# batra-mlp-lab/visdial

Hardware: AMD Instinct MI355X
Metric: QA-rounds/sec training mn-att-ques-im-hist+disc (batch 20x10x100) (higher is better)
Workload: dtype f32 operands and results; the option recurrence multiplies the EXACT 3-way bf16 split of both operands (9 bf16 MFMA products per fp32 product, f32 accumulate: fp32-grade, errors at the f32 MFMA's own level) -- its two step kernels and its weight-gradient contraction; f32 MFMA (v_mfma_f32_32x32x2_f32

## Files before the change

visdial_amd/csrc/comm.hip:

```cpp
#include <dlfcn.h>

#include "common.h"
#include "rt_core.h"
#include "../../include/visdial_hip.h"

namespace {

struct NcclUniqueId { char internal[128]; };
typedef void* NcclComm;
typedef int NcclResult;
enum { kNcclFloat32 = 7, kNcclSum = 0 };

struct Rccl {
  void* lib = nullptr;
  NcclResult (*GetUniqueId)(NcclUniqueId*) = nullptr;
  NcclResult (*CommInitRank)(NcclComm*, int, NcclUniqueId, int) = nullptr;
  NcclResult (*CommDestroy)(NcclComm) = nullptr;
  NcclResult (*AllReduce)(const void*, void*, size_t, int, int, NcclComm, hipStream_t) = nullptr;
  NcclResult (*GroupStart)() = nullptr;
  NcclResult (*GroupEnd)() = nullptr;
  const char* (*GetErrorString)(NcclResult) = nullptr;
  NcclResult (*GetVersion)(int*) = nullptr;
};

// ... 150 lines not shown
int vd_comm_destroy(void) {
  if (!g.comm) return VD_OK;
  if (g.stream) (void)hipStreamSynchronize(g.stream);
  NcclResult r = g.api.CommDestroy(g.comm);
  release_local();
  if (r != 0) {
    vd_set_error("vd_comm_destroy: ncclCommDestroy -> %s", g.api.GetErrorString(r));
    return VD_ERR_HIP;
  }
  return VD_OK;
}

int vd_model_allreduce_grads(vd_model* m) {
  VdRange r("vd_model_allreduce_grads");
  VD_CHECK_ARG(m, "vd_model_allreduce_grads: null model");
  VD_CHECK_ARG(g.comm, "vd_model_allreduce_grads: no communicator (vd_comm_init first)");
  VD_CHECK_ARG(m->cur >= 0, "vd_model_allreduce_grads: no backward pass has been enqueued");
  int dev = -1;
  VD_HIP(hipGetDevice(&dev));
  VD_CHECK_ARG(dev == g.device, "vd_model_allreduce_grads: communicator lives on device %d, current device is %d", g.device, dev);
  int64_t lo = 0, hi = 0;
  int rc = vd_model_encoder_range(m, &lo, &hi);
  if (rc != VD_OK) return rc;
  const bool split = hi > lo && m->enc_grads_recorded;
  if (split) {
    VD_HIP(hipStreamWaitEvent(g.stream, m->ev_enc_grads, 0));
    VD_NCCL(g.api.AllReduce(m->G + lo, m->G + lo, (size_t)(hi - lo), kNcclFloat32, kNcclSum, g.comm, g.stream));
    VD_HIP(hipEventRecord(g.ev_b1, g.stream));
    VD_HIP(hipEventRecord(g.ev_tail_t, m->s_main));
  }
  g.timed = split;
  VD_HIP(hipEventRecord(g.ev_tail, m->s_main));
  VD_HIP(hipStreamWaitEvent(g.stream, g.ev_tail, 0));
  if (split) {
    VD_NCCL(g.api.GroupStart());
    NcclResult r = 0;
    if (lo > 0) r = g.api.AllReduce(m->G, m->G, (size_t)lo, kNcclFloat32, kNcclSum, g.comm, g.stream);
    if (r == 0 && m->numel > hi)
      r = g.api.AllReduce(m->G + hi, m->G + hi, (size_t)(m->numel - hi), kNcclFloat32, kNcclSum, g.comm, g.stream);
    NcclResult rend = g.api.GroupEnd();
    if (r != 0 || rend != 0) {
      vd_set_error("vd_model_allreduce_grads: bucket 2 -> %s", g.api.GetErrorString(r != 0 ? r : rend));
      return VD_ERR_HIP;
    }
  } else {
    VD_NCCL(g.api.AllReduce(m->G, m->G, (size_t)m->numel, kNcclFloat32, kNcclSum, g.comm, g.stream));
// ... 12 lines not shown
```

visdial_amd/csrc/rt_core.h:

```cpp
#pragma once
#include <math.h>
#include <stdarg.h>
#include <stdlib.h>
#include <string.h>

#include <algorithm>
#include <map>
#include <memory>
#include <numeric>
#include <random>
#include <string>
#include <vector>

#include "../../include/visdial_hip.h"
#include "common.h"
#include "paths.h"
#include "rt_switches.h"
#include "wgrad_plan.h"

static_assert(VD_OK == 0 && VD_ERR_ARG == -1, "rt_switches.h returns the two as literals: it includes no common.h");

int vd_lstm2_forward_p(const vd_lstm2_fwd_t* st, int nstacks, int H, int flags, hipStream_t stream);
int vd_lstm2_backward_p(const vd_lstm2_bwd_t* st, int nstacks, int H, int flags, hipStream_t stream);

int vd_img_drop_gather(const float* pre, const uint8_t* mask1, float* xdrop, int N, int R, int S2, int H, float scale, hipStream_t stream);
int vd_img_common_forward_p(const float* pre, const uint8_t* mask1, const float* xdrop, const float* Wc, const float* bc, const float* qc,
                            const uint8_t* mask2, float* iqc, int N, int R, int S2, int H, int Kc, float scale, int flags, hipStream_t stream);
int vd_img_tr_backward_p(const float* dz, const float* Wc, const float* p, const float* datt, const uint8_t* mask1, float* dpre, int N, int R,
                         int S2, int H, int Kc, float scale, int flags, hipStream_t stream);
int vd_img_common_wgrad_p(const float* dz, const float* pre, const uint8_t* mask1, const float* xdrop, float* dWc, int N, int R, int S2, int H,
                          int Kc, float scale, int flags, hipStream_t stream);

int vd_img_att_forward_p(const float* iqc, const float* wa, const float* ba, const float* pre, const uint8_t* mask1, const float* u0, float* p,
                         float* u1, int N, int R, int S2, int H, int Kc, float scale, const int32_t* cnt, hipStream_t stream);
int vd_img_att_backward_p(float* iqc_dz, const float* wa, const float* pre, const uint8_t* mask1, const uint8_t* mask2, const float* p,
                          const float* datt, float* dwa, float* dba, float* dqc, float* work, int N, int R, int S2, int H, int Kc, float scale,
                          const int32_t* cnt, hipStream_t stream);

int vd_mn_attention_round_p(const float* Q, int64_t q_ld, const float* Hm, float* P, float* hAtt, float* Qout, int B, int R, int r, int H,
                            hipStream_t stream);
int vd_hrea_attention_round_p(const float* sq, const float* sh, const float* Hm, float* P, float* att, int B, int R, int r, int H,
// ... 185 lines not shown
}

struct vd_model {
  vd_model_params p;
  int flags = 0;
  std::string enc_name, dec_name;
  std::vector<vdrt::Tensor> spec;
  std::map<std::string, int> index;
  long numel = 0;
  float *W = nullptr, *G = nullptr, *M = nullptr, *V = nullptr;
  std::map<std::string, vdrt::DevBuf> ws;
  std::map<std::string, vdrt::DevBuf> ext_masks;
  hipStream_t s_main = nullptr, s_side = nullptr;
  hipStream_t s_wg = nullptr;
  bool wg_active = false, wg_used = false;
  std::vector<vdrt::WgradProduct> wgrad;
  bool wgrad_open = false, wgrad_hold = false;
  std::vector<hipEvent_t> ev_pool;
  size_t ev_next = 0;
  hipEvent_t ev_enc_grads = nullptr;
  hipEvent_t ev_updated = nullptr;
  bool updated_recorded = false;
  bool enc_grads_recorded = false;
  hipEvent_t ev_loss = nullptr, ev_prof[6] = {nullptr, nullptr, nullptr, nullptr, nullptr, nullptr};
  bool training = true, streams = true, prof_valid = false;
  long step = 0;
  int adam_t = 0;
  double lr = 1e-3;
  vdrt::BatchSlot slot[2];
  int cur = -1, uploaded = -1;
  float* loss_host = nullptr;
  long loss_cap = 0, loss_n = 0;
  bool loss_is_sum = false;
  double loss_div = 0.0;
  std::unique_ptr<vdrt::Encoder> enc;
  std::unique_ptr<vdrt::Decoder> dec;
  float* scores = nullptr;
  float* gen_enc_out = nullptr;
  int gen_seq_len = 0;
  int N = 0, O = 0;
  long lhood_exec = -1, lhood_total = 0;
  bool step_live = false;
  bool use_im = false, use_hist = false, is_att = false, is_graph = false;
  vdrt::OptionCache ocache;
  vdrt::Switches sw;
  int rollout_max_words = 0;
// ... 30 lines not shown
}

template <class T>
int ws_get(vd_model* m, const std::string& key, size_t count, T** out) {
  void* p = nullptr;
  VD_TRY(dev_get(m->ws, key, count * sizeof(T), &p));
  *out = static_cast<T*>(p);
  return VD_OK;
}

inline void add_lstm(vd_model* m, const std::string& name, long D, long H) {
  m->spec.push_back(Tensor{name + ".W", 0, D + H, 4 * H, 1});
  m->spec.push_back(Tensor{name + ".b", 0, 1, 4 * H, 2});
}
inline void add_linear(vd_model* m, const std::string& name, long in, long out) {
  m->spec.push_back(Tensor{name + ".W", 0, out, in, 3});
  m->spec.push_back(Tensor{name + ".b", 0, 1, out, 4});
}
inline std::string hop_sfx(int i) { return i == 0 ? std::string() : std::to_string(i + 1); }

inline float* Wp(vd_model* m, const std::string& n) { return m->W + m->spec[m->index.at(n)].off; }
inline float* Gp(vd_model* m, const std::string& n) { return m->G + m->spec[m->index.at(n)].off; }

inline int fork_stream(vd_model* m, hipStream_t from, hipStream_t side) {
  if (side == from) return VD_OK;
  hipEvent_t e = m->ev_pool[m->ev_next++ % m->ev_pool.size()];
  VD_HIP(hipEventRecord(e, from));
  VD_HIP(hipStreamWaitEvent(side, e, 0));
  return VD_OK;
}
inline int join_stream(vd_model* m, hipStream_t side, hipStream_t to) { return fork_stream(m, side, to); }
inline hipStream_t side_stream(vd_model* m, hipStream_t cur) { return m->streams ? m->s_side : cur; }
inline int wg_fork(vd_model* m, hipStream_t cur, hipStream_t* out) {
  *out = cur;
  if (!m->wg_active || !m->s_wg) return VD_OK;
  VD_TRY(fork_stream(m, cur, m->s_wg));
  m->wg_used = true;
  *out = m->s_wg;
  return VD_OK;
}

constexpr int VD_WGRAD_CHUNKS = 768, VD_WGRAD_MIN_KSTEPS = 32;
inline void wgrad_begin(vd_model* m) {
  m->wgrad.clear();
  m->wgrad_open = true;
}
// ... 359 lines not shown
```

visdial_amd/csrc/rt_decoders.h:

```cpp
#pragma once
#include "rt_encoders.h"

namespace vdrt {

int option_cache_resolve(vd_model* m, BatchSlot& sl, const int32_t* options, long NO, int To, hipStream_t s);

struct Decoder {
  virtual ~Decoder() {}
  virtual void declare(vd_model* m) = 0;
  virtual int forward_backward(vd_model* m, BatchSlot& b, bool only_forward) = 0;
  virtual int retrieve(vd_model* m, BatchSlot& b) = 0;
  virtual int retrieve_lhood(vd_model*, BatchSlot&) {
    vd_set_error("vd_model_retrieve_lhood: the live-row log-likelihood head scores candidates of decoder 'gen'; this model's decoder is 'disc'");
    return VD_ERR_ARG;
  }
  virtual int gen_begin(vd_model*, const int32_t*, int) { return no_gen(); }
  virtual int gen_step(vd_model*, const int32_t*, float*) { return no_gen(); }
  virtual int gen_select(vd_model*, const int32_t*, int) { return no_gen(); }
  virtual int gen_beam_search(vd_model*, int, int, int, int, int32_t*, double*) { return no_gen(); }
  virtual int gen_sample(vd_model*, int, int, int, double, const double*, int32_t*, double*) { return no_gen(); }
  static int no_gen() {
    vd_set_error("sampling / beam search only for the generative decoder (model.lua:436-438)");
    return VD_ERR_STATE;
  }
// ... 20 lines not shown
               "state of the first: under training-mode dropout the passes would not describe one model; call vd_model_set_training(0) first",
               call);
  return VD_ERR_STATE;
}
inline int rollout_encode(vd_model* m, hipStream_t s, BatchSlot& b, int r, float** enc_out) {
  return m->sw.rollout_round ? m->enc->forward_round(m, s, b, r, enc_out) : m->enc->forward(m, s, b, enc_out);
}
struct HistRows {
  int32_t *tok, *tok_sorted, *inv;
  explicit HistRows(BatchSlot& b) : tok(b.h.tok), tok_sorted(b.h.sorted ? b.h.tok_sorted : nullptr), inv(b.h.sorted ? b.h.inv : nullptr) {}
};

#ifdef VD_PROBE_PHASES
inline hipEvent_t* probe_events() {
  static hipEvent_t e[6];
  static bool made = false;
  if (!made) { for (auto& x : e) (void)hipEventCreate(&x); made = true; }
  return e;
}
#define VD_PROBE_REC(i, stream) (void)hipEventRecord(probe_events()[i], stream)
#else
#define VD_PROBE_REC(i, stream)
#endif
struct Disc : Decoder {
  void declare(vd_model* m) override { add_lstm(m, "opt", m->p.embedSize, m->p.rnnHiddenSize); }
  struct OptStates {
    bool c16;
    float *table, *gates, *h, *c, *h_last;
    vd_bf16_bits *gates16, *h16;
    const float* optH;
  };
  int option_states(vd_model* m, const SeqTok& opt, OptStates* o) {
    const int NO = opt.N, To = opt.T;
    const long H = m->p.rnnHiddenSize, E = m->p.embedSize, V = m->p.vocabSize;
    hipStream_t s = m->s_main;
    VD_TRY(ws_get(m, "opt.table", (size_t)(V + 1) * 4 * H, &o->table));
    VD_TRY(ws_get(m, "opt.gates", (size_t)To * NO * 4 * H, &o->gates));
    VD_TRY(ws_get(m, "opt.h", (size_t)To * NO * H, &o->h));
    VD_TRY(ws_get(m, "opt.c", (size_t)To * NO * H, &o->c));
    float* Wopt = Wp(m, "opt.W");
    const int flags = m->flags;
    VD_TRY(vd_gemm_nn(Wp(m, "embed"), E, Wopt, 4 * H, Wp(m, "opt.b"), o->table, 4 * H, (int)V + 1, (int)(4 * H), (int)E, 0, s));
    o->c16 = (flags & VD_FLAG_BF16) && vd_lstm_c16_fits(NO, (int)H);
    o->gates16 = reinterpret_cast<vd_bf16_bits*>(o->gates);
    o->h16 = reinterpret_cast<vd_bf16_bits*>(o->h);
    o->h_last = nullptr;
    vd_bf16_bits* table16 = nullptr;
    if (o->c16) {
      float* t16;
      VD_TRY(ws_get(m, "opt.table16", (size_t)(V + 1) * 2 * H, &t16));
      VD_TRY(ws_get(m, "opt.h_last", (size_t)NO * H, &o->h_last));
      table16 = reinterpret_cast<vd_bf16_bits*>(t16);
      VD_TRY(vd_f32_to_bf16(o->table, table16, (V + 1) * 4 * H, s));
    }
    VD_HIP(hipEventRecord(m->ev_prof[0], s));
    {
      VdRange r("disc: option LSTM forward");
      if (o->c16) VD_TRY(vd_lstm_forward_c16(table16, 4 * H, opt.tok, Wopt + E * 4 * H, o->gates16, o->h16, o->h_last, o->c, To, NO, (int)H, s));
      else VD_TRY(vd_lstm_forward(o->table, 0, 4 * H, opt.tok, nullptr, Wopt + E * 4 * H, nullptr, nullptr, o->gates, o->h, o->c, To, NO, (int)H, flags, s));
    }
    VD_HIP(hipEventRecord(m->ev_prof[1], s));
    o->optH = o->c16 ? o->h_last : o->h + (long)(To - 1) * NO * H;
    return VD_OK;
  }
  int option_states_full(vd_model* m, BatchSlot& b, const OptStates& o, const float** optH) {
    *optH = o.optH;
    if (!b.opt_uid) return VD_OK;
    const long NOfull = (long)b.q.N * m->p.numOptions, H = m->p.rnnHiddenSize;
    float* full;
    VD_TRY(ws_get(m, "opt.h_full", (size_t)NOfull * H, &full));
    VD_TRY(vd_embed_gather(o.optH, b.opt_uid, nullptr, full, NOfull, (int)H, 1.f, m->s_main));
    *optH = full;
    return VD_OK;
  }
  int forward_backward(vd_model* m, BatchSlot& b, bool only_forward) override {
    VD_CHECK_ARG(b.opt.present, "decoder 'disc' needs batch.options");
    VD_CHECK_ARG(only_forward || b.has_gt, "training decoder 'disc' needs batch.answer_ind");
// ... 95 lines not shown
    VdRange rwg("disc: table gradient + dWh");
    VD_TRY(fork_stream(m, s, sd));
    if (!m->wgrad.empty()) {
      VD_TRY(wgrad_flush(m, b, sd));
      VD_HIP(hipEventRecord(m->ev_enc_grads, sd));
    }
    if (c16) VD_TRY(vd_segment_rowsum_acc_bf16(gates16, 4 * H, opt.tok, perm, (long)To * NO, (int)(4 * H), dtab, 4 * H, sd));
    else VD_TRY(vd_segment_rowsum_acc(gates, 4 * H, opt.tok, perm, (long)To * NO, (int)(4 * H), dtab, 4 * H, sd));
    VD_TRY(vd_colsum_acc(dtab, 4 * H, (int)V + 1, (int)(4 * H), Gp(m, "opt.b"), sd));
    VD_TRY(vd_gemm_tn_acc(Wp(m, "embed"), E, dtab, 4 * H, Gp(m, "opt.W"), 4 * H, (int)E, (int)(4 * H), (int)V + 1, 0, sd));
    VD_HIP(hipEventRecord(m->ev_prof[4], s));
    if (To > 1 && c16)
      VD_TRY(vd_gemm_tn_acc_bf16(h16, gates16 + (long)NO * 4 * H, Gp(m, "opt.W") + E * 4 * H, 4 * H, (int)H, (int)(4 * H), (To - 1) * NO, s));
    else if (To > 1)
      VD_TRY(vd_gemm_tn_acc(h, H, gates + (long)NO * 4 * H, 4 * H, Gp(m, "opt.W") + E * 4 * H, 4 * H, (int)H, (int)(4 * H), (To - 1) * NO,
                            flags & (VD_FLAG_BF16 | VD_FLAG_SPLIT9), s));
    VD_HIP(hipEventRecord(m->ev_prof[5], s));
    VD_TRY(vd_gemm_nt(dtab, 4 * H, Wopt, 4 * H, nullptr, Gp(m, "embed"), E, (int)V + 1, (int)E, (int)(4 * H), VD_ACT_NONE, 2, sd));
    VD_PROBE_REC(3, sd);
    VD_TRY(join_stream(m, sd, s));
    if (m->wg_used) VD_TRY(join_stream(m, m->s_wg, s));
    m->wg_active = m->wg_used = false;
    VD_PROBE_REC(4, s);
    return VD_OK;
  }
  int retrieve(vd_model* m, BatchSlot& b) override {
    if (m->sw.retrieve_rollout && m->use_hist) return retrieve_rollout(m, b);
    return forward_backward(m, b, true);
  }

  int retrieve_rollout(vd_model* m, BatchSlot& b) {
    VD_TRY(refuse_round_rollout_in_training(m, "vd_model_retrieve"));
    if (m->training) {
      vd_set_error("vd_model_retrieve: this model was created with VD_RETRIEVE_ROLLOUT = 1, and a rollout re-runs the encoder once per round: "
                   "under training-mode dropout the passes would not describe one model; call vd_model_set_training(0) first");
      return VD_ERR_STATE;
    }
    VD_CHECK_ARG(b.opt.present && !b.cached, "decoder 'disc' needs batch.options");
    const int N = b.q.N, O = m->p.numOptions, NOfull = N * O, NO = b.opt.N, R = m->p.maxQuesCount, B = N / R;
    const bool dedup = b.opt_uid != nullptr;
    VD_CHECK_ARG(dedup ? NO <= NOfull : NO == NOfull, "decoder 'disc': %d option rows for %d x %d candidates", NO, N, O);
    VD_CHECK_ARG(b.h.present && b.q.present && b.h.N == N && N == B * R && b.h.T >= b.q.T,
                 "vd_model_retrieve: VD_RETRIEVE_ROLLOUT = 1 needs the batch's history, Th >= Tq");
    const long H = m->p.rnnHiddenSize;
    hipStream_t s = m->s_main;
    hipStream_t sd = side_stream(m, s);
// ... 17 lines not shown
      if (r > 0) {
        VdRange rr("encoder forward");
        VD_TRY(rollout_encode(m, s, b, r, &enc_out));
      }
      VD_TRY(vd_score_ce(optH, enc_out, b.gt, scores, loss_rows, nullptr, nullptr, N, O, (int)H, 1.0f / N, s));
      if (r + 1 < R)
        VD_TRY(vd_disc_rollout_pick_p(scores, O, b.opt.tok, NO, b.opt.T, b.opt_uid, b.q.tok, b.q.T, B, R, r, hr.tok, hr.tok_sorted, hr.inv,
                                      b.h.T, s, m->sw.rollout_concat_end));
    }
    VD_TRY(stage_loss(m, loss_rows, N, false, s));
    m->scores = scores;
    m->prof_valid = false;
    return VD_OK;
  }

  int forward_cached(vd_model* m, BatchSlot& b, bool only_forward) {
    if (!only_forward || m->training) {
      vd_set_error("decoder 'disc': this batch was uploaded for cached evaluation (VD_OPTION_CACHE with training off) and carries only the "
                   "candidate rows the cache did not hold; upload it again after vd_model_set_training(1) for a training step");
      return VD_ERR_STATE;
    }
    OptionCache& oc = m->ocache;
    const int N = b.q.N, O = m->p.numOptions, NOfull = N * O, To = b.opt.T;
    const long H = m->p.rnnHiddenSize, E = m->p.embedSize, V = m->p.vocabSize;
    hipStream_t s = m->s_main;
    hipStream_t sd = side_stream(m, s);
    if (b.cache_stamp != oc.stamp) {
      VD_HIP(hipEventSynchronize(b.ready));
      VD_TRY(option_cache_resolve(m, b, b.opt_host.data(), NOfull, To, s));
      VD_HIP(hipStreamSynchronize(s));
    }
    const int U = b.opt.N;
    const long count = oc.index.size();
    VD_CHECK_ARG(b.opt_total == NOfull && (long)b.miss_keys.size() == (long)U * To && count <= oc.capacity,
                 "decoder 'disc': inconsistent cached batch (%d candidates, %d misses)", b.opt_total, U);
    if (oc.table_rows < count + U) {
      const long want = std::min(std::max(2 * oc.table_rows, VD_OPTION_CACHE_FIRST_ROWS), oc.capacity);
      const long rows = std::max(want, count + U);
      float* nt = nullptr;
      VD_HIP(hipMalloc((void**)&nt, (size_t)rows * H * sizeof(float)));
      if (oc.table) {
        if (count > 0) VD_HIP(hipMemcpyAsync(nt, oc.table, (size_t)count * H * sizeof(float), hipMemcpyDeviceToDevice, s));
        VD_HIP(hipStreamSynchronize(s));
        VD_HIP(hipFree(oc.table));
      }
      oc.table = nt;
      oc.table_rows = rows;
    }
    float *scores, *loss_rows, *full;
    VD_TRY(ws_get(m, "opt.scores", (size_t)N * O, &scores));
    VD_TRY(ws_get(m, "crit.loss_rows", (size_t)N, &loss_rows));
    VD_TRY(ws_get(m, "opt.h_full", (size_t)NOfull * H, &full));
    VD_TRY(fork_stream(m, s, sd));
    if (U > 0) {
      VdRange r("disc: option LSTM forward (state only, cache misses)");
      float *table, *h, *c;
      VD_TRY(ws_get(m, "opt.table", (size_t)(V + 1) * 4 * H, &table));
      VD_TRY(ws_get(m, "opt.h2", (size_t)2 * U * H, &h));
      VD_TRY(ws_get(m, "opt.c2", (size_t)2 * U * H, &c));
      float* Wopt = Wp(m, "opt.W");
      VD_TRY(vd_gemm_nn(Wp(m, "embed"), E, Wopt, 4 * H, Wp(m, "opt.b"), table, 4 * H, (int)V + 1, (int)(4 * H), (int)E, 0, s));
      VD_TRY(vd_lstm_forward(table, 0, 4 * H, b.opt.tok, nullptr, Wopt + E * 4 * H, nullptr, nullptr, nullptr, h, c, To, U, (int)H,
                             m->flags | VD_FLAG_STATE_ONLY, s));
      VD_HIP(hipMemcpyAsync(oc.table + count * H, h + (long)((To - 1) & 1) * U * H, (size_t)U * H * sizeof(float), hipMemcpyDeviceToDevice, s));
      const long fit = std::min<long>(U, oc.capacity - count);
      for (long i = 0; i < fit; ++i) oc.index.add(b.miss_keys.data() + (size_t)i * To);
    }
    ++oc.stamp;
    float* enc_out = nullptr;
    {
      VdRange r("encoder forward");
      VD_TRY(m->enc->forward(m, sd, b, &enc_out));
    }
    VD_TRY(join_stream(m, sd, s));
    VD_TRY(vd_embed_gather(oc.table, b.opt_uid, nullptr, full, NOfull, (int)H, 1.f, s));
    VD_TRY(vd_score_ce(full, enc_out, b.gt, scores, loss_rows, nullptr, nullptr, N, O, (int)H, 1.0f / N, s));
    VD_TRY(stage_loss(m, loss_rows, N, false, s));
    m->scores = scores;
    m->prof_valid = false;
    return VD_OK;
  }
};

struct Gen;
// ... 585 lines not shown
```

visdial_amd/csrc/runtime.hip:

```cpp
#include "rt_decoders.h"

using namespace vdrt;

vd_model::~vd_model() {}

namespace {

int upload_tokens(BatchSlot& sl, SeqTok& ss, const std::string& tag, const int32_t* rows_major, int N, int T, bool sorted, hipStream_t s,
                  int rollout_R = 0) {
  ss.T = T;
  ss.N = N;
  ss.present = true;
  ss.sorted = sorted;
  sl.wgrad_sig.clear();
  const size_t TN = (size_t)T * N;
  const size_t seg_at = (7 * TN + 2 * (size_t)N + T + 3) / 4 * 4, seg_ints = 4 * ((size_t)T + 1);
  const size_t total = sorted ? seg_at + 2 * seg_ints : TN;
  int32_t* stage = nullptr;
  VD_TRY(pin_get(sl.pinned, tag + ".stage", total * sizeof(int32_t), (void**)&stage));
  int32_t* tok = stage;
  std::vector<int> len(sorted ? N : 0);
  for (int n = 0; n < N; ++n) {
    int first = T;
    for (int t = 0; t < T; ++t) {
// ... 258 lines not shown
  m->ocache.capacity = sw.option_cache_rows;
  if (m->p.numAttentionLayers < 1 || has(en, "lf-att")) m->p.numAttentionLayers = 1;
  if (m->p.numLayers < 1) m->p.numLayers = 2;
  m->enc_name = encoder;
  m->dec_name = decoder;
  m->use_im = use_im;
  m->use_hist = has(en, "hist");
  m->is_att = is_att;
  m->is_graph = en.rfind("mn", 0) == 0 || en.rfind("lf-att", 0) == 0;
  m->lr = p->learningRate;
  m->streams = p->useStreams != 0;
  m->enc = std::move(enc);
  m->dec = std::move(dec);
  m->spec.push_back(Tensor{"embed", 0, p->vocabSize + 1, p->embedSize, 0});
  m->enc->declare(m);
  m->dec->declare(m);
  long off = 0;
  for (size_t i = 0; i < m->spec.size(); ++i) {
    m->spec[i].off = off;
    m->index[m->spec[i].name] = (int)i;
    off += (m->spec[i].numel() + 3) / 4 * 4;
  }
  m->numel = off;
  auto fail = [&](int rc) {
    vd_model_destroy(m);
    return rc;
  };
  for (float** v : {&m->W, &m->G, &m->M, &m->V}) {
    if (hipMalloc((void**)v, off * sizeof(float)) != hipSuccess) {
      vd_set_error("vd_model_create: hipMalloc of %ld floats failed", off);
      return fail(VD_ERR_HIP);
    }
    (void)hipMemset(*v, 0, off * sizeof(float));
  }
  int least = 0, greatest = 0;
  (void)hipDeviceGetStreamPriorityRange(&least, &greatest);
  if (hipStreamCreateWithPriority(&m->s_main, hipStreamNonBlocking, least) != hipSuccess) return fail(VD_ERR_HIP);
  if (hipStreamCreateWithPriority(&m->s_side, hipStreamNonBlocking, greatest) != hipSuccess) return fail(VD_ERR_HIP);
  if (least - greatest >= 2 &&
      hipStreamCreateWithPriority(&m->s_wg, hipStreamNonBlocking, (least + greatest) / 2) != hipSuccess)
    return fail(VD_ERR_HIP);
  m->ev_pool.resize(64);
  for (auto& e : m->ev_pool)
    if (hipEventCreateWithFlags(&e, hipEventDisableTiming) != hipSuccess) return fail(VD_ERR_HIP);
  if (hipEventCreateWithFlags(&m->ev_loss, hipEventDisableTiming) != hipSuccess) return fail(VD_ERR_HIP);
  if (hipEventCreateWithFlags(&m->ev_enc_grads, hipEventDisableTiming) != hipSuccess) return fail(VD_ERR_HIP);
// ... 40 lines not shown
    }
  delete m;
}

int64_t vd_model_num_tensors(const vd_model* m) { return m ? (int64_t)m->spec.size() : 0; }
int64_t vd_model_flat_size(const vd_model* m) { return m ? m->numel : 0; }

int vd_model_tensor_info(const vd_model* m, int64_t i, char* name64, int64_t* offset, int64_t* rows, int64_t* cols) {
  VD_CHECK_ARG(m && i >= 0 && i < (int64_t)m->spec.size(), "vd_model_tensor_info: bad index");
  const Tensor& t = m->spec[i];
  if (name64) {
    strncpy(name64, t.name.c_str(), 63);
    name64[63] = 0;
  }
  if (offset) *offset = t.off;
  if (rows) *rows = t.rows;
  if (cols) *cols = t.cols;
  return VD_OK;
}

int vd_model_flat_pointers(vd_model* m, float** W, float** dW, float** adam_m, float** adam_v) {
  VD_CHECK_ARG(m, "vd_model_flat_pointers: null model");
  m->ocache.flush();
  if (W) *W = m->W;
  if (dW) *dW = m->G;
  if (adam_m) *adam_m = m->M;
  if (adam_v) *adam_v = m->V;
  return VD_OK;
}

void* vd_model_stream(vd_model* m) { return m ? (void*)m->s_main : nullptr; }

int vd_model_encoder_range(const vd_model* m, int64_t* lo, int64_t* hi) {
  VD_CHECK_ARG(m && lo && hi, "vd_model_encoder_range: null");
  const char* first_dec = m->dec_name == "disc" ? "opt.W" : "dec1.W";
  *lo = m->spec[1].off;
  *hi = m->spec[m->index.at(first_dec)].off;
  return VD_OK;
}
int vd_model_wait_encoder_grads(vd_model* m, void* stream) {
  VD_CHECK_ARG(m && m->enc_grads_recorded, "vd_model_wait_encoder_grads: no backward pass has been enqueued");
  VD_HIP(hipStreamWaitEvent((hipStream_t)stream, m->ev_enc_grads, 0));
  return VD_OK;
}

int vd_model_init_params(vd_model* m, uint64_t seed) {
  VD_CHECK_ARG(m, "vd_model_init_params: null model");
  std::mt19937_64 rng(seed);
  std::vector<float> host((size_t)m->numel, 0.f);
  const long H = m->p.rnnHiddenSize;
  for (const Tensor& t : m->spec) {
    float* w = host.data() + t.off;
    const long n = t.numel();
    if (t.kind == 0) {
      std::normal_distribution<float> nd(0.f, 1.f);
      for (long i = t.cols; i < n; ++i) w[i] = nd(rng);
    } else if (t.kind == 1) {
      std::normal_distribution<float> nd(0.f, 1.f / sqrtf((float)t.rows));
      for (long i = 0; i < n; ++i) w[i] = nd(rng);
    } else if (t.kind == 2) {
      for (long i = H; i < 2 * H; ++i) w[i] = 1.f;
    } else {
      const long in = t.kind == 3 ? t.cols : m->spec[m->index.at(t.name.substr(0, t.name.size() - 2) + ".W")].cols;
      const float s = 1.f / sqrtf((float)in);
      std::uniform_real_distribution<float> ud(-s, s);
      for (long i = 0; i < n; ++i) w[i] = ud(rng);
    }
  }
  VD_HIP(hipMemcpy(m->W, host.data(), host.size() * sizeof(float), hipMemcpyHostToDevice));
  m->ocache.flush();
  return VD_OK;
}

static int attach_dense_relevance(vd_model* m, const float* host, int64_t n, bool live) {
  const char* who = live ? "vd_model_set_tensor: '@dense_relevance_live'" : "vd_model_set_tensor: '@dense_relevance'";
  VD_CHECK_ARG(!live || !(m->flags & VD_FLAG_BF16),
               "%s runs the live rounds' candidate rows through the fp32 / split option recurrence; this model was created with lstmBf16 = 1, "
               "whose compact-state recurrence is not covered: attach '@dense_relevance'", who);
  VD_CHECK_ARG(m->uploaded >= 0, "%s attaches to the batch uploaded last, and no batch has been uploaded", who);
  BatchSlot& sl = m->slot[m->uploaded];
  const int N = sl.q.N, O = m->p.numOptions;
  VD_CHECK_ARG(n == (int64_t)N * O, "%s holds N x O = %d x %d = %ld values for this batch, got %ld", who, N, O, (long)N * O, (long)n);
  double W = 0.0;
  std::vector<int32_t> live_idx, live_slot((size_t)N, -1);
  for (int r = 0; r < N; ++r) {
    const float* row = host + (size_t)r * O;
    int minus = 0;
    double sum = 0.0;
    for (int o = 0; o < O; ++o) {
      const float v = row[o];
      VD_CHECK_ARG(v == -1.f || (v >= 0.f && v <= FLT_MAX),
                   "%s row %d, candidate %d = %g: a relevance is finite and >= 0, and a round without an annotation is a full row of -1", who, r,
// ... 86 lines not shown
  double* out;
  VD_TRY(ws_get(m, "ndcg.rows", (size_t)m->N, &out));
  VD_HIP(hipStreamWaitEvent(m->s_main, b.ready, 0));
  VD_TRY(vd_ndcg_p(m->scores, b.rel, out, m->N, m->O, m->s_main));
  VD_HIP(hipMemcpyAsync(host, out, (size_t)m->N * sizeof(double), hipMemcpyDeviceToHost, m->s_main));
  VD_HIP(hipEventRecord(b.done, m->s_main));
  VD_HIP(hipStreamSynchronize(m->s_main));
  return VD_OK;
}

int vd_model_set_tensor(vd_model* m, const char* name, const float* host, int64_t n) {
  if (m && name && host && name[0] == '@') {
    if (!strcmp(name, "@dense_relevance")) return attach_dense_relevance(m, host, n, false);
    if (!strcmp(name, "@dense_relevance_live")) return attach_dense_relevance(m, host, n, true);
    if (!strcmp(name, "@img_regions")) return attach_img_regions(m, host, n);
    VD_CHECK_ARG(false, "vd_model_set_tensor: unknown batch attachment '%s' (the library knows '@dense_relevance' and '@dense_relevance_live') "
                 "and, for the image attention, '@img_regions'", name);
  }
  VD_CHECK_ARG(m && name && host && m->index.count(name), "vd_model_set_tensor: unknown tensor '%s'", name ? name : "(null)");
  const Tensor& t = m->spec[m->index.at(name)];
  VD_CHECK_ARG(n == t.numel(), "vd_model_set_tensor: '%s' holds %ld values, got %ld", name, t.numel(), (long)n);
  VD_HIP(hipStreamSynchronize(m->s_main));
  VD_HIP(hipMemcpy(m->W + t.off, host, n * sizeof(float), hipMemcpyHostToDevice));
  m->ocache.flush();
  return VD_OK;
}

int vd_model_get_tensor(vd_model* m, const char* name, int which, float* host, int64_t n) {
  if (m && name && host && name[0] == '@') {
    if (!strcmp(name, "@ndcg")) return read_ndcg(m, which, host, n);
    VD_CHECK_ARG(false, "vd_model_get_tensor: unknown batch attachment '%s' (the library knows '@ndcg')", name);
  }
  VD_CHECK_ARG(m && name && host && m->index.count(name), "vd_model_get_tensor: unknown tensor '%s'", name ? name : "(null)");
  const Tensor& t = m->spec[m->index.at(name)];
  VD_CHECK_ARG(n == t.numel() && which >= 0 && which <= 3, "vd_model_get_tensor: bad size / selector");
  VD_HIP(hipStreamSynchronize(m->s_main));
  float* base[4] = {m->W, m->G, m->M, m->V};
  VD_HIP(hipMemcpy(host, base[which] + t.off, n * sizeof(float), hipMemcpyDeviceToHost));
  return VD_OK;
}

int vd_model_set_training(vd_model* m, int on) {
  VD_CHECK_ARG(m, "vd_model_set_training: null model");
  m->training = on != 0;
  if (on) m->ocache.flush();
  return VD_OK;
}

int vd_model_set_dropout_mask(vd_model* m, const char* site, const uint8_t* host, int64_t n) {
  VD_CHECK_ARG(m, "vd_model_set_dropout_mask: null model");
  VD_HIP(hipStreamSynchronize(m->s_main));
  if (!host) {
    for (auto& kv : m->ext_masks)
      if (kv.second.p) VD_HIP(hipFree(kv.second.p));
    m->ext_masks.clear();
    return VD_OK;
  }
  VD_CHECK_ARG(site && n > 0, "vd_model_set_dropout_mask: bad arguments");
  void* p = nullptr;
  VD_TRY(dev_get(m->ext_masks, site, (size_t)n, &p));
  VD_HIP(hipMemcpy(p, host, (size_t)n, hipMemcpyHostToDevice));
  return VD_OK;
}

int vd_model_upload_batch(vd_model* m, const vd_batch* hb) {
  VD_CHECK_ARG(m && hb && hb->ques_fwd && hb->B > 0 && hb->Tq > 0, "vd_model_upload_batch: missing ques_fwd / B / Tq");
  VD_CHECK_ARG(!m->use_hist || (hb->hist && hb->Th > 0), "vd_model_upload_batch: encoder '%s' needs hist", m->enc_name.c_str());
  VD_CHECK_ARG(!m->use_im || hb->img_feat, "vd_model_upload_batch: encoder '%s' needs img_feat", m->enc_name.c_str());
// ... 104 lines not shown
    sl.gt_host[n] = g;
    gp[n] = g;
  }
  VD_TRY(dev_get(sl.bufs, "gt", (size_t)N * sizeof(int32_t), (void**)&sl.gt));
  VD_HIP(hipMemcpyAsync(sl.gt, gp, (size_t)N * sizeof(int32_t), hipMemcpyHostToDevice, s));
  VD_HIP(hipEventRecord(sl.ready, s));
  m->uploaded = (int)(&sl - m->slot);
  m->lhood_exec = -1;
  return VD_OK;
}

static int begin_step(vd_model* m, bool zero_grads, BatchSlot** out) {
  VD_CHECK_ARG(m && m->uploaded >= 0, "no batch uploaded");
  m->cur = m->uploaded;
  m->enc_grads_recorded = false;
  m->lhood_exec = -1;
  m->step_live = false;
  BatchSlot& b = m->slot[m->cur];
  m->N = b.q.N;
  m->O = m->p.numOptions;
  hipStream_t s = m->s_main;
  VD_HIP(hipStreamWaitEvent(s, b.ready, 0));
  if (zero_grads) VD_TRY(vd_memset(m->G, 0, m->numel * 4, s));
  VD_TRY(vd_memset(Wp(m, "embed"), 0, (long)m->p.embedSize * 4, s));
  b.used = true;
  *out = &b;
  return VD_OK;
}

int vd_model_forward_backward(vd_model* m, int only_forward) {
  VdRange r(only_forward ? "vd_model_forward" : "vd_model_forward_backward");
  BatchSlot* b = nullptr;
  VD_TRY(begin_step(m, !only_forward, &b));
  if (!only_forward) m->ocache.flush();
  const int rc = m->dec->forward_backward(m, *b, only_forward != 0);
  VD_HIP(hipEventRecord(b->done, m->s_main));
  return rc;
}

int vd_model_retrieve(vd_model* m) {
  VdRange r("vd_model_retrieve");
  BatchSlot* b = nullptr;
  VD_TRY(begin_step(m, false, &b));
  const int rc = m->dec->retrieve(m, *b);
  VD_HIP(hipEventRecord(b->done, m->s_main));
  return rc;
// ... 43 lines not shown
                    int32_t* host_tokens, double* host_loglik) {
  VD_CHECK_ARG(m, "vd_model_sample: null model");
  VdRange r("vd_model_sample");
  return m->dec->gen_sample(m, beam_len, start_token, end_token, temperature, host_uniforms, host_tokens, host_loglik);
}

int vd_model_loss(vd_model* m, float* loss) {
  VD_CHECK_ARG(m && loss && m->cur >= 0 && m->loss_n > 0, "vd_model_loss: nothing to read");
  VD_HIP(hipEventSynchronize(m->ev_loss));
  double s = 0;
  for (long i = 0; i < m->loss_n; ++i) s += m->loss_host[i];
  *loss = (float)(m->loss_is_sum ? s : s / (m->loss_div > 0.0 ? m->loss_div : (double)m->loss_n));
  return VD_OK;
}

int vd_model_update(vd_model* m, float gscale) {
  VD_CHECK_ARG(m, "vd_model_update: null model");
  VdRange r("vd_model_update: clamp + adam");
  m->adam_t += 1;
  m->ocache.flush();
  const double t = m->adam_t;
  const float step = (float)(m->lr * sqrt(1.0 - pow(0.999, t)) / (1.0 - pow(0.9, t)));
  const float clip_norm = (float)m->sw.grad_clip_norm, decay = (float)(m->lr * m->sw.weight_decay);
  if (clip_norm > 0.f || decay > 0.f) {
    float* work = nullptr;
    if (clip_norm > 0.f) {
      VD_TRY(ws_get(m, "upd.clip_work", (size_t)vd_clip_work_floats(), &work));
      VD_TRY(vd_grad_clip_scale_p(m->G, m->numel, gscale, clip_norm, work, m->s_main));
    }
    VD_TRY(vd_clip_decay_adam_p(m->W, m->G, m->M, m->V, m->numel, gscale, 5.0f, 0.9f, 0.999f, 1e-8f, step, work, decay, m->s_main));
  } else {
    VD_TRY(vd_clamp_adam(m->W, m->G, m->M, m->V, m->numel, gscale, 5.0f, 0.9f, 0.999f, 1e-8f, step, m->s_main));
  }
  VD_HIP(hipEventRecord(m->ev_updated, m->s_main));
  m->updated_recorded = true;
  if (m->lr > m->p.minLRate) m->lr *= m->p.lrDecayRate;
  m->step += 1;
  return VD_OK;
}

int vd_model_learning_rate(vd_model* m, double* lr, int set) {
  VD_CHECK_ARG(m && lr, "vd_model_learning_rate: null");
  if (set) m->lr = *lr;
  else *lr = m->lr;
  return VD_OK;
}

int vd_model_scores(vd_model* m, float* host, int64_t n) {
  VD_CHECK_ARG(m && host && m->cur >= 0 && m->scores && n == (int64_t)m->N * m->O, "vd_model_scores: no scores / bad size");
  VD_HIP(hipStreamSynchronize(m->s_main));
  VD_HIP(hipMemcpy(host, m->scores, n * sizeof(float), hipMemcpyDeviceToHost));
  return VD_OK;
}

int vd_model_ranks(vd_model* m, int use_gt, int32_t* ranks_out) {
// ... 58 lines not shown
```

visdial_amd/native.py:

```python
import ctypes as C

import numpy as np

from . import _lib
from .split_eval import SplitEval, rollout_answered_history

call = _lib.call


def _text(v):
    return None if v is None else str(v)


def _int0(v):
    return int(v or 0)


SWITCHES = (
    ('optionCache', 'VD_OPTION_CACHE', lambda v: str(_int0(v)), _int0, 0, None),
    ('fusedLhood', 'VD_LHOOD_TREE', lambda v: '1' if _int0(v) == 2 else '0', _int0, 0, None),
    ('topK', 'VD_SAMPLE_TOPK', _text, int, 0, 'gen'),
    ('topP', 'VD_SAMPLE_TOPP', _text, float, 1.0, 'gen'),
    ('beamGroups', 'VD_BEAM_GROUPS', _text, int, 1, 'gen'),
    ('beamDiversity', 'VD_BEAM_DIVERSITY', _text, float, 0.5, None),
# ... 129 lines not shown
        for name, _, r, c in self.tensors:
            a = np.ascontiguousarray(d[name], dtype=np.float32)
            assert a.size == r * c, name
            call("vd_model_set_tensor", self.h, name.encode(), a.ctypes.data, a.size)

    def _get(self, which):
        out = {}
        for name, _, r, c in self.tensors:
            a = np.empty(self._shape(name, r, c), np.float32)
            call("vd_model_get_tensor", self.h, name.encode(), which, a.ctypes.data, a.size)
            out[name] = a
        return out

    def get_parameters_dict(self):
        return self._get(0)

    def get_gradients_dict(self):
        return self._get(1)

    @property
    def wrapperW(self):
        if self._W is None:
            import torch
            ptrs = [C.c_void_p() for _ in range(4)]
            call("vd_model_flat_pointers", self.h, *[C.byref(x) for x in ptrs])
            n = int(_lib.load().vd_model_flat_size(self.h))
            self._W = torch.as_tensor(_DevArray(ptrs[0].value, n), device='cuda')
        self.synchronize()
        return self._W

    def _entries(self):
        kind = lambda n: 'embed' if n == 'embed' else ('lstm' if n.split('.')[0].rstrip('0123456789') in
                                                        ('hist', 'ques', 'opt', 'dec', 'dialog') else 'lin') + \
            ('_w' if n.endswith('.W') else '_b')
        return [(n, self._shape(n, r, c), kind(n)) for n, _, r, c in self.tensors]

    def load_flat_parameters(self, modelW):
        from . import t7
        self.set_parameters_dict(t7.flat_to_named(np.asarray(modelW), self._entries(), self.params['encoder']))

    def flat_parameters(self):
        from . import t7
        return t7.named_to_flat(self.get_parameters_dict(), self._entries(), self.params['encoder'])

    def training(self, on=True):
        call("vd_model_set_training", self.h, int(on))

    def set_dropout_masks(self, masks):
        call("vd_model_set_dropout_mask", self.h, None, None, 0)
        for k, v in (masks or {}).items():
# ... 255 lines not shown
```

Measured before the change: 9612.

## Rebuild option embedding table during Adam step on side stream, cache by version stamps

Adds per-tensor version stamps so the option input table (embed × opt.W + b) and its bf16 copy are rebuilt only when embed, opt.W or opt.b change. When safe, the Adam update is split: the slices holding embed and opt input weights are updated first on a side stream, then the table is rebuilt there while the rest of the parameters update on the main stream. This takes the table GEMM off the critical path of the next forward. The cost is extra bookkeeping and stream joins. It also needs correct invalidation whenever weights are written elsewhere, such as host pointers, set_tensor or training toggles.

```diff
diff --git a/visdial_amd/csrc/comm.hip b/visdial_amd/csrc/comm.hip
--- a/visdial_amd/csrc/comm.hip
+++ b/visdial_amd/csrc/comm.hip
@@ -196,6 +196,7 @@
   int64_t lo = 0, hi = 0;
   int rc = vd_model_encoder_range(m, &lo, &hi);
   if (rc != VD_OK) return rc;
+  m->grads_reduced = true;
   const bool split = hi > lo && m->enc_grads_recorded;
   if (split) {
     VD_HIP(hipStreamWaitEvent(g.stream, m->ev_enc_grads, 0));
diff --git a/visdial_amd/csrc/param_stamp.h b/visdial_amd/csrc/param_stamp.h
--- /dev/null
+++ b/visdial_amd/csrc/param_stamp.h
@@ -0,0 +1,66 @@
+#pragma once
+#include <cstdint>
+#include <vector>
+
+namespace vdstamp {
+
+struct Dep {
+  int tensor, part;
+};
+
+struct Versions {
+  std::vector<uint64_t> v;
+  uint64_t clock = 0;
+  void init(size_t tensors) { v.assign(2 * tensors, 0), clock = 0; }
+  uint64_t get(Dep d) const { return v[2 * (size_t)d.tensor + d.part]; }
+  void bump(Dep d) { v[2 * (size_t)d.tensor + d.part] = ++clock; }
+  void bump_tensor(int t) { bump(Dep{t, 0}), bump(Dep{t, 1}); }
+  void bump_all() {
+    for (auto& x : v) x = ++clock;
+  }
+  void bump_range(long lo, long hi, const long* off, const long* numel, const long* split, int tensors) {
+    for (int t = 0; t < tensors; ++t) {
+      const long a = off[t], s = off[t] + split[t], b = off[t] + numel[t];
+      if (lo < s && hi > a) bump(Dep{t, 0});
+      if (lo < b && hi > s) bump(Dep{t, 1});
+    }
+  }
+};
+
+struct Stamp {
+  std::vector<uint64_t> built;
+  bool valid = false;
+  bool current(const Versions& ver, const Dep* deps, int n) const {
+    if (!valid || (int)built.size() != n) return false;
+    for (int i = 0; i < n; ++i)
+      if (built[i] != ver.get(deps[i])) return false;
+    return true;
+  }
+  void record(const Versions& ver, const Dep* deps, int n) {
+    built.resize(n);
+    for (int i = 0; i < n; ++i) built[i] = ver.get(deps[i]);
+    valid = true;
+  }
+  void clear() { valid = false; }
+};
+
+struct Range {
+  long lo, hi;
+  long n() const { return hi - lo; }
+};
+struct SlicePlan {
+  Range side[2], main;
+};
+inline SlicePlan slice_plan(long off_optW, long E, long H, long off_optb, long numel) {
+  const long cut = off_optW + E * 4 * H;
+  return SlicePlan{{Range{0, cut}, Range{off_optb, numel}}, Range{cut, off_optb}};
+}
+
+struct StepFacts {
+  bool streams, disc_chain_step, global_clip, reduced_elsewhere, host_holds_grads, bf16_pass;
+};
+inline bool can_slice(const StepFacts& f) {
+  return f.streams && f.disc_chain_step && !f.global_clip && !f.reduced_elsewhere && !f.host_holds_grads && !f.bf16_pass;
+}
+
+}
diff --git a/visdial_amd/csrc/rt_core.h b/visdial_amd/csrc/rt_core.h
--- a/visdial_amd/csrc/rt_core.h
+++ b/visdial_amd/csrc/rt_core.h
@@ -17,6 +17,7 @@
 #include "paths.h"
 #include "rt_switches.h"
 #include "wgrad_plan.h"
+#include "param_stamp.h"
 
 static_assert(VD_OK == 0 && VD_ERR_ARG == -1, "rt_switches.h returns the two as literals: it includes no common.h");
 
@@ -248,6 +249,9 @@
   hipEvent_t ev_updated = nullptr;
   bool updated_recorded = false;
   bool enc_grads_recorded = false;
+  vdstamp::Versions ver;
+  vdstamp::Stamp table_stamp, table16_stamp;
+  bool chain_step = false, grads_reduced = false, host_grads = false;
   hipEvent_t ev_loss = nullptr, ev_prof[6] = {nullptr, nullptr, nullptr, nullptr, nullptr, nullptr};
   bool training = true, streams = true, prof_valid = false;
   long step = 0;
@@ -324,6 +328,19 @@
 inline float* Wp(vd_model* m, const std::string& n) { return m->W + m->spec[m->index.at(n)].off; }
 inline float* Gp(vd_model* m, const std::string& n) { return m->G + m->spec[m->index.at(n)].off; }
 
+inline void mark_written(vd_model* m, long lo, long hi) {
+  const int n = (int)m->spec.size();
+  std::vector<long> off(n), numel(n), split(n);
+  for (int i = 0; i < n; ++i) {
+    const Tensor& t = m->spec[i];
+    off[i] = t.off, numel[i] = t.numel();
+    split[i] = t.kind == 1 ? (t.rows - t.cols / 4) * t.cols : t.numel();
+  }
+  m->ver.bump_range(lo, hi, off.data(), numel.data(), split.data(), n);
+}
+inline void mark_all_written(vd_model* m) { m->ver.bump_all(); }
+inline vdstamp::Dep dep_of(vd_model* m, const std::string& n, int part) { return vdstamp::Dep{m->index.at(n), part}; }
+
 inline int fork_stream(vd_model* m, hipStream_t from, hipStream_t side) {
   if (side == from) return VD_OK;
   hipEvent_t e = m->ev_pool[m->ev_next++ % m->ev_pool.size()];
diff --git a/visdial_amd/csrc/rt_decoders.h b/visdial_amd/csrc/rt_decoders.h
--- a/visdial_amd/csrc/rt_decoders.h
+++ b/visdial_amd/csrc/rt_decoders.h
@@ -66,6 +66,27 @@
 #else
 #define VD_PROBE_REC(i, stream)
 #endif
+inline int option_table(vd_model* m, hipStream_t s, bool want16, float** table, vd_bf16_bits** table16) {
+  const long H = m->p.rnnHiddenSize, E = m->p.embedSize, V = m->p.vocabSize;
+  const vdstamp::Dep deps[3] = {dep_of(m, "embed", 0), dep_of(m, "opt.W", 0), dep_of(m, "opt.b", 0)};
+  VD_TRY(ws_get(m, "opt.table", (size_t)(V + 1) * 4 * H, table));
+  if (!m->table_stamp.current(m->ver, deps, 3)) {
+    VD_TRY(vd_gemm_nn(Wp(m, "embed"), E, Wp(m, "opt.W"), 4 * H, Wp(m, "opt.b"), *table, 4 * H, (int)V + 1, (int)(4 * H), (int)E, 0, s));
+    m->table_stamp.record(m->ver, deps, 3);
+    m->table16_stamp.clear();
+  }
+  if (table16) *table16 = nullptr;
+  if (!want16) return VD_OK;
+  float* t16;
+  VD_TRY(ws_get(m, "opt.table16", (size_t)(V + 1) * 2 * H, &t16));
+  if (!m->table16_stamp.current(m->ver, deps, 3)) {
+    VD_TRY(vd_f32_to_bf16(*table, reinterpret_cast<vd_bf16_bits*>(t16), (V + 1) * 4 * H, s));
+    m->table16_stamp.record(m->ver, deps, 3);
+  }
+  if (table16) *table16 = reinterpret_cast<vd_bf16_bits*>(t16);
+  return VD_OK;
+}
+
 struct Disc : Decoder {
   void declare(vd_model* m) override { add_lstm(m, "opt", m->p.embedSize, m->p.rnnHiddenSize); }
   struct OptStates {
@@ -76,27 +97,20 @@
   };
   int option_states(vd_model* m, const SeqTok& opt, OptStates* o) {
     const int NO = opt.N, To = opt.T;
-    const long H = m->p.rnnHiddenSize, E = m->p.embedSize, V = m->p.vocabSize;
+    const long H = m->p.rnnHiddenSize, E = m->p.embedSize;
     hipStream_t s = m->s_main;
-    VD_TRY(ws_get(m, "opt.table", (size_t)(V + 1) * 4 * H, &o->table));
     VD_TRY(ws_get(m, "opt.gates", (size_t)To * NO * 4 * H, &o->gates));
     VD_TRY(ws_get(m, "opt.h", (size_t)To * NO * H, &o->h));
     VD_TRY(ws_get(m, "opt.c", (size_t)To * NO * H, &o->c));
     float* Wopt = Wp(m, "opt.W");
     const int flags = m->flags;
-    VD_TRY(vd_gemm_nn(Wp(m, "embed"), E, Wopt, 4 * H, Wp(m, "opt.b"), o->table, 4 * H, (int)V + 1, (int)(4 * H), (int)E, 0, s));
     o->c16 = (flags & VD_FLAG_BF16) && vd_lstm_c16_fits(NO, (int)H);
     o->gates16 = reinterpret_cast<vd_bf16_bits*>(o->gates);
     o->h16 = reinterpret_cast<vd_bf16_bits*>(o->h);
     o->h_last = nullptr;
     vd_bf16_bits* table16 = nullptr;
-    if (o->c16) {
-      float* t16;
-      VD_TRY(ws_get(m, "opt.table16", (size_t)(V + 1) * 2 * H, &t16));
-      VD_TRY(ws_get(m, "opt.h_last", (size_t)NO * H, &o->h_last));
-      table16 = reinterpret_cast<vd_bf16_bits*>(t16);
-      VD_TRY(vd_f32_to_bf16(o->table, table16, (V + 1) * 4 * H, s));
-    }
+    VD_TRY(option_table(m, s, o->c16, &o->table, &table16));
+    if (o->c16) VD_TRY(ws_get(m, "opt.h_last", (size_t)NO * H, &o->h_last));
     VD_HIP(hipEventRecord(m->ev_prof[0], s));
     {
       VdRange r("disc: option LSTM forward");
@@ -238,6 +252,7 @@
     if (m->wg_used) VD_TRY(join_stream(m, m->s_wg, s));
     m->wg_active = m->wg_used = false;
     VD_PROBE_REC(4, s);
+    m->chain_step = true;
     return VD_OK;
   }
   int retrieve(vd_model* m, BatchSlot& b) override {
@@ -301,7 +316,7 @@
     }
     OptionCache& oc = m->ocache;
     const int N = b.q.N, O = m->p.numOptions, NOfull = N * O, To = b.opt.T;
-    const long H = m->p.rnnHiddenSize, E = m->p.embedSize, V = m->p.vocabSize;
+    const long H = m->p.rnnHiddenSize, E = m->p.embedSize;
     hipStream_t s = m->s_main;
     hipStream_t sd = side_stream(m, s);
     if (b.cache_stamp != oc.stamp) {
@@ -334,11 +349,10 @@
     if (U > 0) {
       VdRange r("disc: option LSTM forward (state only, cache misses)");
       float *table, *h, *c;
-      VD_TRY(ws_get(m, "opt.table", (size_t)(V + 1) * 4 * H, &table));
+      VD_TRY(option_table(m, s, false, &table, nullptr));
       VD_TRY(ws_get(m, "opt.h2", (size_t)2 * U * H, &h));
       VD_TRY(ws_get(m, "opt.c2", (size_t)2 * U * H, &c));
       float* Wopt = Wp(m, "opt.W");
-      VD_TRY(vd_gemm_nn(Wp(m, "embed"), E, Wopt, 4 * H, Wp(m, "opt.b"), table, 4 * H, (int)V + 1, (int)(4 * H), (int)E, 0, s));
       VD_TRY(vd_lstm_forward(table, 0, 4 * H, b.opt.tok, nullptr, Wopt + E * 4 * H, nullptr, nullptr, nullptr, h, c, To, U, (int)H,
                              m->flags | VD_FLAG_STATE_ONLY, s));
       VD_HIP(hipMemcpyAsync(oc.table + count * H, h + (long)((To - 1) & 1) * U * H, (size_t)U * H * sizeof(float), hipMemcpyDeviceToDevice, s));
diff --git a/visdial_amd/csrc/runtime.hip b/visdial_amd/csrc/runtime.hip
--- a/visdial_amd/csrc/runtime.hip
+++ b/visdial_amd/csrc/runtime.hip
@@ -304,6 +304,7 @@
     off += (m->spec[i].numel() + 3) / 4 * 4;
   }
   m->numel = off;
+  m->ver.init(m->spec.size());
   auto fail = [&](int rc) {
     vd_model_destroy(m);
     return rc;
@@ -390,6 +391,8 @@
 int vd_model_flat_pointers(vd_model* m, float** W, float** dW, float** adam_m, float** adam_v) {
   VD_CHECK_ARG(m, "vd_model_flat_pointers: null model");
   m->ocache.flush();
+  mark_all_written(m);
+  if (dW) m->host_grads = true;
   if (W) *W = m->W;
   if (dW) *dW = m->G;
   if (adam_m) *adam_m = m->M;
@@ -408,6 +411,7 @@
 }
 int vd_model_wait_encoder_grads(vd_model* m, void* stream) {
   VD_CHECK_ARG(m && m->enc_grads_recorded, "vd_model_wait_encoder_grads: no backward pass has been enqueued");
+  m->grads_reduced = true;
   VD_HIP(hipStreamWaitEvent((hipStream_t)stream, m->ev_enc_grads, 0));
   return VD_OK;
 }
@@ -436,6 +440,7 @@
     }
   }
   VD_HIP(hipMemcpy(m->W, host.data(), host.size() * sizeof(float), hipMemcpyHostToDevice));
+  mark_all_written(m);
   m->ocache.flush();
   return VD_OK;
 }
@@ -568,6 +573,7 @@
   VD_CHECK_ARG(n == t.numel(), "vd_model_set_tensor: '%s' holds %ld values, got %ld", name, t.numel(), (long)n);
   VD_HIP(hipStreamSynchronize(m->s_main));
   VD_HIP(hipMemcpy(m->W + t.off, host, n * sizeof(float), hipMemcpyHostToDevice));
+  mark_written(m, t.off, t.off + t.numel());
   m->ocache.flush();
   return VD_OK;
 }
@@ -590,6 +596,7 @@
   VD_CHECK_ARG(m, "vd_model_set_training: null model");
   m->training = on != 0;
   if (on) m->ocache.flush();
+  if (on) mark_all_written(m);
   return VD_OK;
 }
 
@@ -740,6 +747,7 @@
   hipStream_t s = m->s_main;
   VD_HIP(hipStreamWaitEvent(s, b.ready, 0));
   if (zero_grads) VD_TRY(vd_memset(m->G, 0, m->numel * 4, s));
+  m->chain_step = m->grads_reduced = false;
   VD_TRY(vd_memset(Wp(m, "embed"), 0, (long)m->p.embedSize * 4, s));
   b.used = true;
   *out = &b;
@@ -829,15 +837,43 @@
   const double t = m->adam_t;
   const float step = (float)(m->lr * sqrt(1.0 - pow(0.999, t)) / (1.0 - pow(0.9, t)));
   const float clip_norm = (float)m->sw.grad_clip_norm, decay = (float)(m->lr * m->sw.weight_decay);
-  if (clip_norm > 0.f || decay > 0.f) {
+  const vdstamp::StepFacts facts{m->streams && m->s_side != nullptr, m->chain_step, clip_norm > 0.f, m->grads_reduced, m->host_grads,
+                                 (m->flags & VD_FLAG_BF16) != 0};
+  m->chain_step = m->grads_reduced = false;
+  if (vdstamp::can_slice(facts)) {
+    const long E = m->p.embedSize, H = m->p.rnnHiddenSize;
+    const vdstamp::SlicePlan plan = vdstamp::slice_plan(m->spec[m->index.at("opt.W")].off, E, H, m->spec[m->index.at("opt.b")].off, m->numel);
+    auto slice = [&](vdstamp::Range r, hipStream_t s) -> int {
+      if (decay > 0.f)
+        VD_TRY(vd_clip_decay_adam_p(m->W + r.lo, m->G + r.lo, m->M + r.lo, m->V + r.lo, r.n(), gscale, 5.0f, 0.9f, 0.999f, 1e-8f, step, nullptr, decay, s));
+      else
+        VD_TRY(vd_clamp_adam(m->W + r.lo, m->G + r.lo, m->M + r.lo, m->V + r.lo, r.n(), gscale, 5.0f, 0.9f, 0.999f, 1e-8f, step, s));
+      mark_written(m, r.lo, r.hi);
+      return VD_OK;
+    };
+    hipStream_t sd = m->s_side;
+    VD_HIP(hipStreamWaitEvent(sd, m->ev_enc_grads, 0));
+    VD_TRY(slice(plan.side[0], sd));
+    VD_TRY(slice(plan.side[1], sd));
+    float *table, *pad;
+    VD_TRY(ws_get(m, "upd.pad_row", (size_t)E, &pad));
+    VD_HIP(hipMemcpyAsync(pad, Wp(m, "embed"), (size_t)E * 4, hipMemcpyDeviceToDevice, sd));
+    VD_TRY(vd_memset(Wp(m, "embed"), 0, E * 4, sd));
+    VD_TRY(option_table(m, sd, false, &table, nullptr));
+    VD_HIP(hipMemcpyAsync(Wp(m, "embed"), pad, (size_t)E * 4, hipMemcpyDeviceToDevice, sd));
+    VD_TRY(slice(plan.main, m->s_main));
+    VD_TRY(join_stream(m, sd, m->s_main));
+  } else if (clip_norm > 0.f || decay > 0.f) {
     float* work = nullptr;
     if (clip_norm > 0.f) {
       VD_TRY(ws_get(m, "upd.clip_work", (size_t)vd_clip_work_floats(), &work));
       VD_TRY(vd_grad_clip_scale_p(m->G, m->numel, gscale, clip_norm, work, m->s_main));
     }
     VD_TRY(vd_clip_decay_adam_p(m->W, m->G, m->M, m->V, m->numel, gscale, 5.0f, 0.9f, 0.999f, 1e-8f, step, work, decay, m->s_main));
+    mark_all_written(m);
   } else {
     VD_TRY(vd_clamp_adam(m->W, m->G, m->M, m->V, m->numel, gscale, 5.0f, 0.9f, 0.999f, 1e-8f, step, m->s_main));
+    mark_all_written(m);
   }
   VD_HIP(hipEventRecord(m->ev_updated, m->s_main));
   m->updated_recorded = true;
diff --git a/visdial_amd/native.py b/visdial_amd/native.py
--- a/visdial_amd/native.py
+++ b/visdial_amd/native.py
@@ -175,10 +175,10 @@
     def wrapperW(self):
         if self._W is None:
             import torch
-            ptrs = [C.c_void_p() for _ in range(4)]
-            call("vd_model_flat_pointers", self.h, *[C.byref(x) for x in ptrs])
+            ptr = C.c_void_p()
+            call("vd_model_flat_pointers", self.h, C.byref(ptr), None, None, None)
             n = int(_lib.load().vd_model_flat_size(self.h))
-            self._W = torch.as_tensor(_DevArray(ptrs[0].value, n), device='cuda')
+            self._W = torch.as_tensor(_DevArray(ptr.value, n), device='cuda')
         self.synchronize()
         return self._W
 
```

Result: no change. 9595 (-0.2%).
